# kowaalczyk/reformer-tts

Measured on AMD Instinct MI355X. Metric: mel-frames/sec training step, LJSpeech-shape batch, higher is better.
Workload: dtype bf16; 1 GPU; config/baseline.yml full Reformer-TTS training step (enc 3 / dec 3 layers, d=512, LSH 8 rounds, buckets 64/128), per-GPU batch 12, text 200->256, mel 1024x80; global_batch=12, parallelism=dp1, reversible_recompute=full

## Files before the change

### reformer-tts_amd/csrc/edges.hip

```cpp
#include "rtts_common.h"

#define ED_THREADS 256
#define ED_PBLOCKS 256

#define ed_drop rtts_drop_keep

struct EdHalo {
    int B, L, P, H;
};
__device__ __forceinline__ bool ed_valid(const EdHalo& g, long long m, int& b, int& t) {
    if (m < 0 || m >= (long long)g.B * g.P) return false;
    const int mi = (int)m;
    int q = (int)((float)mi * __builtin_amdgcn_rcpf((float)g.P));
    int r = mi - q * g.P;
    if (r < 0) { --q; r += g.P; }
    if (r >= g.P) { ++q; r -= g.P; }
    b = q;
    t = r - g.H;
    return (unsigned)t < (unsigned)g.L;
}
__device__ __forceinline__ void ed_row_col(unsigned e, int C, int cshift, unsigned& row, int& c) {
    if (cshift >= 0) {
        row = e >> cshift;
        c = (int)(e & (unsigned)(C - 1));
    } else {
        row = e / (unsigned)C;
        c = (int)(e - row * (unsigned)C);
    }
}
static inline int ed_cshift(int C) { return (C & (C - 1)) == 0 ? __builtin_ctz((unsigned)C) : -1; }
__device__ __forceinline__ float ed_tanh(float x) {
    const float t = __builtin_amdgcn_exp2f(x * 2.885390081777927f);
    return 1.f - 2.f * __builtin_amdgcn_rcpf(t + 1.f);
}
static inline EdHalo ed_halo(int B, int L, int halo) { return EdHalo{B, L, L + 2 * halo, halo}; }

template <bool SRC_F32>
__global__ __launch_bounds__(ED_THREADS) void to_halo_kernel(const void* __restrict__ src, int64_t ld_src, int64_t bs_src, int C_src, EdHalo g, int C,
                                                             int lead, long long rows, bf16_t* __restrict__ dst) {
    const int pieces = C / 8;
    const size_t total = (size_t)rows * pieces;
    for (size_t i = (size_t)blockIdx.x * blockDim.x + threadIdx.x; i < total; i += (size_t)gridDim.x * blockDim.x) {
        const int pc = (int)(i % pieces);
        const long long r = (long long)(i / pieces);
        int b, t;
        uint4 o = make_uint4(0, 0, 0, 0);
        if (pc * 8 < C_src && ed_valid(g, r - lead, b, t)) {
            const size_t soff = (size_t)b * bs_src + (size_t)t * ld_src;
            if (SRC_F32) {
                const float* p = reinterpret_cast<const float*>(src) + soff + pc * 8;
                const float4 v0 = *reinterpret_cast<const float4*>(p), v1 = *reinterpret_cast<const float4*>(p + 4);
                o.x = pack_bf16x2(v0.x, v0.y); o.y = pack_bf16x2(v0.z, v0.w);
                o.z = pack_bf16x2(v1.x, v1.y); o.w = pack_bf16x2(v1.z, v1.w);
            } else {
                o = *reinterpret_cast<const uint4*>(reinterpret_cast<const bf16_t*>(src) + soff + pc * 8);
            }
        }
        *reinterpret_cast<uint4*>(dst + (size_t)r * C + pc * 8) = o;
    }
}

__global__ __launch_bounds__(ED_THREADS) void conv_w_perm_kernel(const float* __restrict__ w, int Co, int Ci, int CP, bf16_t* __restrict__ wp) {
    const size_t total = (size_t)Co * 5 * CP;
    for (size_t i = (size_t)blockIdx.x * blockDim.x + threadIdx.x; i < total; i += (size_t)gridDim.x * blockDim.x) {
        const int ci = (int)(i % CP), k = (int)((i / CP) % 5), co = (int)(i / ((size_t)CP * 5));
        wp[i] = ci < Ci ? f32_to_bf16(w[((size_t)co * Ci + ci) * 5 + k]) : (bf16_t)0;
    }
}
struct CwGroup {
    rtts_conv_perm_job j[RTTS_CONV_PERM_MAX_GROUP];
    int blk_start[RTTS_CONV_PERM_MAX_GROUP + 1];
    int n;
};
__global__ __launch_bounds__(ED_THREADS) void conv_w_perm_grouped_kernel(const CwGroup g) {
    int ji = 0;
#pragma unroll
    for (int i = 1; i < RTTS_CONV_PERM_MAX_GROUP; ++i)
        if (i < g.n && (int)blockIdx.x >= g.blk_start[i]) ji = i;
    const rtts_conv_perm_job& J = g.j[ji];
    const int Co = J.Co, Ci = J.Ci, CP = J.CP;
    const float* __restrict__ w = J.w;
    bf16_t* __restrict__ wp = (bf16_t*)J.wp;
    const size_t total = (size_t)Co * CP;
    const size_t nthr = (size_t)(g.blk_start[ji + 1] - g.blk_start[ji]) * blockDim.x;
    for (size_t i = (size_t)((int)blockIdx.x - g.blk_start[ji]) * blockDim.x + threadIdx.x; i < total; i += nthr) {
        const int ci = (int)(i % CP), co = (int)(i / CP);
        float t[5] = {0.f, 0.f, 0.f, 0.f, 0.f};
        if (ci < Ci) {
            const float* src = w + ((size_t)co * Ci + ci) * 5;
#pragma unroll
            for (int k = 0; k < 5; ++k) t[k] = src[k];
        }
#pragma unroll
        for (int k = 0; k < 5; ++k) wp[((size_t)co * 5 + k) * CP + ci] = f32_to_bf16(t[k]);
    }
}
__global__ __launch_bounds__(ED_THREADS) void conv_dw_unperm_grouped_kernel(const CwGroup g) {
    int ji = 0;
#pragma unroll
    for (int i = 1; i < RTTS_CONV_PERM_MAX_GROUP; ++i)
        if (i < g.n && (int)blockIdx.x >= g.blk_start[i]) ji = i;
    const rtts_conv_perm_job& J = g.j[ji];
    const int Co = J.Co, Ci = J.Ci, CP = J.CP;
    const float* __restrict__ dwp = J.w;
    float* __restrict__ dw = (float*)J.wp;
    const size_t total = (size_t)Co * Ci;
    const size_t nthr = (size_t)(g.blk_start[ji + 1] - g.blk_start[ji]) * blockDim.x;
    for (size_t i = (size_t)((int)blockIdx.x - g.blk_start[ji]) * blockDim.x + threadIdx.x; i < total; i += nthr) {
        const int ci = (int)(i % Ci), co = (int)(i / Ci);
        float* dst = dw + i * 5;
#pragma unroll
        for (int k = 0; k < 5; ++k) dst[k] += dwp[((size_t)co * 5 + k) * CP + ci];
    }
}
__global__ __launch_bounds__(ED_THREADS) void conv_dw_unperm_kernel(const float* __restrict__ dwp, int Co, int Ci, int CP, float* __restrict__ dw) {
    const size_t total = (size_t)Co * Ci * 5;
    for (size_t i = (size_t)blockIdx.x * blockDim.x + threadIdx.x; i < total; i += (size_t)gridDim.x * blockDim.x) {
        const int k = (int)(i % 5), ci = (int)((i / 5) % Ci), co = (int)(i / ((size_t)Ci * 5));
        dw[i] += dwp[((size_t)co * 5 + k) * CP + ci];
    }
}

template <int MODE>
__global__ __launch_bounds__(ED_THREADS) void col_partial_kernel(const float* __restrict__ y, const bf16_t* __restrict__ dz,
                                                                 const float* __restrict__ mean, const float* __restrict__ rstd,
                                                                 const float* __restrict__ gamma, const float* __restrict__ beta, int act,
                                                                 uint32_t seed, const uint32_t* __restrict__ seed_dev, uint32_t thresh, float dscale, EdHalo g,
                                                                 int dz_halo, int C, float* __restrict__ partial) {
    if (seed_dev) seed += seed_dev[0];
    const int M = g.B * g.P;
    const int cq = threadIdx.x & 63, rl = threadIdx.x >> 6;
    const int c = blockIdx.y * 256 + cq * 4;
    __shared__ float red[2][4][256];
    float sa[4] = {0, 0, 0, 0}, sb[4] = {0, 0, 0, 0};
    if (c < C) {
        float mu[4] = {0, 0, 0, 0}, rs[4] = {1, 1, 1, 1}, ga[4] = {1, 1, 1, 1}, be[4] = {0, 0, 0, 0};
        if (MODE == 1) {
#pragma unroll
            for (int j = 0; j < 4; ++j) { mu[j] = mean[c + j]; rs[j] = rstd[c + j]; ga[j] = gamma[c + j]; be[j] = beta[c + j]; }
        }
        for (int row = blockIdx.x * 4 + rl; row < M; row += gridDim.x * 4) {
            int sb_, st_;
            if (!ed_valid(g, row, sb_, st_)) continue;
            const float4 yv = *reinterpret_cast<const float4*>(y + (size_t)row * C + c);
            const float yy[4] = {yv.x, yv.y, yv.z, yv.w};
            if (MODE == 0) {
#pragma unroll
                for (int j = 0; j < 4; ++j) { sa[j] += yy[j]; sb[j] = __builtin_fmaf(yy[j], yy[j], sb[j]); }
            } else {
                const size_t drow = dz_halo ? (size_t)row : (size_t)sb_ * g.L + st_;
                const uint2 dv = *reinterpret_cast<const uint2*>(dz + drow * C + c);
                const float dd[4] = {__uint_as_float(dv.x << 16), __uint_as_float(dv.x & 0xffff0000u), __uint_as_float(dv.y << 16),
                                     __uint_as_float(dv.y & 0xffff0000u)};
#pragma unroll
                for (int j = 0; j < 4; ++j) {
                    const float yh = (yy[j] - mu[j]) * rs[j];
                    const float pre = __builtin_fmaf(yh, ga[j], be[j]);
                    float da;
                    if (act == 1) da = pre > 0.f ? 1.f : 0.f;
                    else { const float th = ed_tanh(pre); da = 1.f - th * th; }
                    const float g = dd[j] * da * (thresh ? ed_drop(seed, (uint32_t)((size_t)row * C + c + j), thresh, dscale) : 1.f);
                    sa[j] += g;
                    sb[j] = __builtin_fmaf(g, yh, sb[j]);
                }
            }
        }
    }
#pragma unroll
    for (int j = 0; j < 4; ++j) { red[0][rl][cq * 4 + j] = sa[j]; red[1][rl][cq * 4 + j] = sb[j]; }
    __syncthreads();
    const int t = threadIdx.x;
    if (blockIdx.y * 256 + t < C) {
        float* prow = partial + (size_t)blockIdx.x * 2 * C;
        prow[blockIdx.y * 256 + t] = (red[0][0][t] + red[0][1][t]) + (red[0][2][t] + red[0][3][t]);
        prow[C + blockIdx.y * 256 + t] = (red[1][0][t] + red[1][1][t]) + (red[1][2][t] + red[1][3][t]);
    }
}

#define ED_FIN_WAVES 16
__device__ __forceinline__ void ed_reduce_partials(const float* __restrict__ partial, int nrows, int C, int c, float& s, float& q,
                                                   float (*red)[ED_FIN_WAVES][64]) {
    const int lane = threadIdx.x & 63, wave = threadIdx.x >> 6;
    float a = 0.f, b = 0.f;
    if (c < C) {
        float va[16], vb[16];
        for (int r0 = wave; r0 < nrows; r0 += ED_FIN_WAVES * 16) {
#pragma unroll
            for (int u = 0; u < 16; ++u) {
                const int r = r0 + u * ED_FIN_WAVES;
                va[u] = r < nrows ? partial[(size_t)r * 2 * C + c] : 0.f;
                vb[u] = r < nrows ? partial[(size_t)r * 2 * C + C + c] : 0.f;
            }
#pragma unroll
            for (int u = 0; u < 16; ++u) {
                a += va[u];
                b += vb[u];
            }
        }
    }
    red[0][wave][lane] = a;
    red[1][wave][lane] = b;
    __syncthreads();
    s = 0.f;
    q = 0.f;
#pragma unroll
    for (int w = 0; w < ED_FIN_WAVES; ++w) {
        s += red[0][w][lane];
        q += red[1][w][lane];
    }
}

__global__ __launch_bounds__(64 * ED_FIN_WAVES) void bn_finalize_stats_kernel(const float* __restrict__ partial, int nrows, int M, int C,
                                                                       float* __restrict__ mean, float* __restrict__ rstd,
                                                                       float* __restrict__ run_mean, float* __restrict__ run_var,
                                                                       const float* __restrict__ mean_shift, long long* __restrict__ num_batches) {
    __shared__ float red[2][ED_FIN_WAVES][64];
    const int c = blockIdx.x * 64 + (threadIdx.x & 63);
    float s, q;
    ed_reduce_partials(partial, nrows, C, c, s, q, red);
    if (num_batches && blockIdx.x == 0 && threadIdx.x == 0) num_batches[0] += 1;
    if (threadIdx.x >= 64 || c >= C) return;
    const float mu = s / M;
    const float var = fmaxf(q / M - mu * mu, 0.f);
    mean[c] = mu;
    rstd[c] = rsqrtf(var + 1e-5f);
    if (run_mean) {
        run_mean[c] = 0.9f * run_mean[c] + 0.1f * (mu + (mean_shift ? mean_shift[c] : 0.f));
        run_var[c] = 0.9f * run_var[c] + 0.1f * var * ((float)M / (float)(M > 1 ? M - 1 : 1));
    }
}

__global__ __launch_bounds__(64 * ED_FIN_WAVES) void bn_finalize_bwd_kernel(const float* __restrict__ partial, int nrows, int C,
                                                                     float* __restrict__ sums, float* __restrict__ dgamma,
                                                                     float* __restrict__ dbeta) {
    __shared__ float red[2][ED_FIN_WAVES][64];
    const int c = blockIdx.x * 64 + (threadIdx.x & 63);
    float s, q;
    ed_reduce_partials(partial, nrows, C, c, s, q, red);
    if (threadIdx.x >= 64 || c >= C) return;
    sums[c] = s;
    sums[C + c] = q;
    dbeta[c] += s;
    dgamma[c] += q;
}

__global__ __launch_bounds__(64 * ED_FIN_WAVES) void bn_moments_kernel(const float* __restrict__ partial, int nrows, int C, float* __restrict__ moments) {
    __shared__ float red[2][ED_FIN_WAVES][64];
    const int c = blockIdx.x * 64 + (threadIdx.x & 63);
    float s, q;
    ed_reduce_partials(partial, nrows, C, c, s, q, red);
    if (threadIdx.x >= 64 || c >= C) return;
    moments[c] = s;
    moments[C + c] = q;
}
__global__ void bn_from_moments_kernel(const float* __restrict__ moments, float count, int C, float* __restrict__ mean, float* __restrict__ rstd,
                                       float* __restrict__ run_mean, float* __restrict__ run_var, const float* __restrict__ mean_shift,
                                       long long* __restrict__ num_batches) {
    const int c = blockIdx.x * blockDim.x + threadIdx.x;
    if (num_batches && c == 0) num_batches[0] += 1;
    if (c >= C) return;
    if (count <= 0.f) count = moments[2 * C];
    const float mu = moments[c] / count;
    const float var = fmaxf(moments[C + c] / count - mu * mu, 0.f);
    mean[c] = mu;
    rstd[c] = rsqrtf(var + 1e-5f);
    if (run_mean) {
        run_mean[c] = 0.9f * run_mean[c] + 0.1f * (mu + (mean_shift ? mean_shift[c] : 0.f));
        run_var[c] = 0.9f * run_var[c] + 0.1f * var * (count / (count > 1.f ? count - 1.f : 1.f));
    }
}

__global__ __launch_bounds__(ED_THREADS) void bn_act_fwd_kernel(const float* __restrict__ y, const float* __restrict__ mean,
                                                                const float* __restrict__ rstd, const float* __restrict__ gamma,
                                                                const float* __restrict__ beta, int act, uint32_t seed, const uint32_t* __restrict__ seed_dev,
                                                                uint32_t thresh, float dscale, EdHalo g, int z_halo, int z_lead, size_t n4, int C,
                                                                int cshift, bf16_t* __restrict__ z) {
    if (seed_dev) seed += seed_dev[0];
    for (size_t i = (size_t)blockIdx.x * blockDim.x + threadIdx.x; i < n4; i += (size_t)gridDim.x * blockDim.x) {
        unsigned zrow;
        int c;
        ed_row_col((unsigned)i * 4u, C, cshift, zrow, c);
        const long long zr = (long long)zrow;
        long long ym;
        bool ok = true;
        if (z_halo) {
            int b, t;
            ym = zr - z_lead;
            ok = ed_valid(g, ym, b, t);
        } else {
            const long long b = zr / g.L;
            ym = b * g.P + g.H + (zr - b * g.L);
        }
        uint2 pk = make_uint2(0u, 0u);
        if (ok) {
            const size_t e = (size_t)ym * C + c;
            const float4 yv = *reinterpret_cast<const float4*>(y + e);
            const float yy[4] = {yv.x, yv.y, yv.z, yv.w};
            const float4 m4 = *reinterpret_cast<const float4*>(mean + c), r4 = *reinterpret_cast<const float4*>(rstd + c);
            const float4 g4 = *reinterpret_cast<const float4*>(gamma + c), b4 = *reinterpret_cast<const float4*>(beta + c);
            const float mu[4] = {m4.x, m4.y, m4.z, m4.w}, rs[4] = {r4.x, r4.y, r4.z, r4.w};
            const float ga[4] = {g4.x, g4.y, g4.z, g4.w}, be[4] = {b4.x, b4.y, b4.z, b4.w};
            float o[4];
#pragma unroll
            for (int j = 0; j < 4; ++j) {
                const float pre = __builtin_fmaf((yy[j] - mu[j]) * rs[j], ga[j], be[j]);
                float a = act == 1 ? fmaxf(pre, 0.f) : ed_tanh(pre);
                if (thresh) a *= ed_drop(seed, (uint32_t)(e + j), thresh, dscale);
                o[j] = a;
            }
            pk.x = pack_bf16x2(o[0], o[1]);
            pk.y = pack_bf16x2(o[2], o[3]);
        }
        reinterpret_cast<uint2*>(z)[i] = pk;
    }
}

__global__ __launch_bounds__(ED_THREADS) void bn_act_bwd_apply_kernel(const float* __restrict__ y, const bf16_t* __restrict__ dz,
                                                                      const float* __restrict__ mean, const float* __restrict__ rstd,
                                                                      const float* __restrict__ gamma, const float* __restrict__ beta, int act,
// ... 764 lines not shown
```

### reformer-tts_amd/csrc/fused_rows.hip

```cpp
#include "rtts_common.h"

#define FR_THREADS 256
#define FR_WAVES 4
#define FR_PARTIAL_BLOCKS 256

template <int VEC> struct VecF32;
template <> struct VecF32<2> { typedef float2 T; };
template <> struct VecF32<4> { typedef float4 T; };

template <int EPL, int VEC>
__device__ __forceinline__ void load_row_f32(const float* __restrict__ row, int lane, float* v) {
#pragma unroll
    for (int k = 0; k < EPL / VEC; ++k) {
        const typename VecF32<VEC>::T t = *reinterpret_cast<const typename VecF32<VEC>::T*>(row + (k * 64 + lane) * VEC);
        const float* f = reinterpret_cast<const float*>(&t);
#pragma unroll
        for (int j = 0; j < VEC; ++j) v[k * VEC + j] = f[j];
    }
}

template <int EPL, int VEC>
__device__ __forceinline__ void store_row_f32(float* __restrict__ row, int lane, const float* v) {
#pragma unroll
    for (int k = 0; k < EPL / VEC; ++k) {
        typename VecF32<VEC>::T t;
        float* f = reinterpret_cast<float*>(&t);
#pragma unroll
        for (int j = 0; j < VEC; ++j) f[j] = v[k * VEC + j];
        *reinterpret_cast<typename VecF32<VEC>::T*>(row + (k * 64 + lane) * VEC) = t;
    }
}

#ifndef RTTS_ROW_WT
#define RTTS_ROW_WT 0
#endif
template <int EPL, int VEC>
__device__ __forceinline__ void store_row_f32_out(float* __restrict__ row, int lane, const float* v) {
#if RTTS_ROW_WT >= 1
    if constexpr (VEC == 4) {
#pragma unroll
        for (int k = 0; k < EPL / VEC; ++k) {
            uint4 t;
            t.x = __float_as_uint(v[k * 4]); t.y = __float_as_uint(v[k * 4 + 1]); t.z = __float_as_uint(v[k * 4 + 2]); t.w = __float_as_uint(v[k * 4 + 3]);
            rtts_store16_out(row + (k * 64 + lane) * 4, t);
        }
        return;
    }
#endif
    store_row_f32<EPL, VEC>(row, lane, v);
}

template <int EPL, int VEC>
__device__ __forceinline__ void load_row_bf16(const bf16_t* __restrict__ row, int lane, float* v) {
#pragma unroll
    for (int k = 0; k < EPL / VEC; ++k) {
        const bf16_t* p = row + (k * 64 + lane) * VEC;
        if constexpr (VEC == 8) {
            const uint4 t = *reinterpret_cast<const uint4*>(p);
            const uint32_t u[4] = {t.x, t.y, t.z, t.w};
#pragma unroll
            for (int j = 0; j < 4; ++j) {
                v[k * 8 + 2 * j] = __uint_as_float(u[j] << 16);
                v[k * 8 + 2 * j + 1] = __uint_as_float(u[j] & 0xffff0000u);
            }
        } else if constexpr (VEC == 4) {
            const uint2 t = *reinterpret_cast<const uint2*>(p);
            v[k * 4] = __uint_as_float(t.x << 16);
            v[k * 4 + 1] = __uint_as_float(t.x & 0xffff0000u);
            v[k * 4 + 2] = __uint_as_float(t.y << 16);
            v[k * 4 + 3] = __uint_as_float(t.y & 0xffff0000u);
        } else {
            const uint32_t t = *reinterpret_cast<const uint32_t*>(p);
            v[k * 2] = __uint_as_float(t << 16);
            v[k * 2 + 1] = __uint_as_float(t & 0xffff0000u);
        }
    }
}

template <int EPL, int VEC, bool WT = true>
__device__ __forceinline__ void store_row_bf16(bf16_t* __restrict__ row, int lane, const float* v) {
#pragma unroll
    for (int k = 0; k < EPL / VEC; ++k) {
        bf16_t* p = row + (k * 64 + lane) * VEC;
        if constexpr (VEC == 8) {
            uint4 t;
            t.x = pack_bf16x2(v[k * 8], v[k * 8 + 1]);
            t.y = pack_bf16x2(v[k * 8 + 2], v[k * 8 + 3]);
            t.z = pack_bf16x2(v[k * 8 + 4], v[k * 8 + 5]);
            t.w = pack_bf16x2(v[k * 8 + 6], v[k * 8 + 7]);
            *reinterpret_cast<uint4*>(p) = t;
        } else if constexpr (VEC == 4) {
            uint2 t;
            t.x = pack_bf16x2(v[k * 4], v[k * 4 + 1]);
            t.y = pack_bf16x2(v[k * 4 + 2], v[k * 4 + 3]);
#if RTTS_ROW_WT >= 2
            if (WT) {
                typedef int rv2i __attribute__((ext_vector_type(2)));
                const rv2i w2 = {(int)t.x, (int)t.y};
                asm volatile("global_store_dwordx2 %0, %1, off sc1" ::"v"(p), "v"(w2) : "memory");
                continue;
            }
#endif
            *reinterpret_cast<uint2*>(p) = t;
        } else {
            *reinterpret_cast<uint32_t*>(p) = pack_bf16x2(v[k * 2], v[k * 2 + 1]);
        }
    }
}

template <int VEC>
__device__ __forceinline__ int row_col(int e, int lane) { return ((e / VEC) * 64 + lane) * VEC + (e % VEC); }

__device__ __forceinline__ float wave_sum(float s) {
#pragma unroll
    for (int o = 32; o > 0; o >>= 1) s += __shfl_xor(s, o);
    return s;
}

template <int EPL, int VEC>
__device__ __forceinline__ void block_partial(const float* acc, float* __restrict__ partial_row, float* lds) {
    const int lane = threadIdx.x & 63, wave = threadIdx.x >> 6;
    store_row_f32<EPL, VEC>(lds + wave * EPL * 64, lane, acc);
    __syncthreads();
    for (int c = threadIdx.x; c < EPL * 64; c += FR_THREADS)
        partial_row[c] = lds[c] + lds[EPL * 64 + c] + lds[2 * EPL * 64 + c] + lds[3 * EPL * 64 + c];
    __syncthreads();
}

template <int EPL, int VEC>
__global__ __launch_bounds__(FR_THREADS) void ln_fwd_kernel(const float* __restrict__ x, const float* __restrict__ gamma,
                                                            const float* __restrict__ beta, bf16_t* __restrict__ xn,
                                                            float* __restrict__ mean, float* __restrict__ rstd, int M) {
    constexpr int D = EPL * 64;
    const int lane = threadIdx.x & 63;
    const int row = blockIdx.x * FR_WAVES + (threadIdx.x >> 6);
    if (row >= M) return;
    float v[EPL], g[EPL], b[EPL];
    load_row_f32<EPL, VEC>(x + (size_t)row * D, lane, v);
    load_row_f32<EPL, VEC>(gamma, lane, g);
    load_row_f32<EPL, VEC>(beta, lane, b);
    float s = 0.f;
#pragma unroll
    for (int e = 0; e < EPL; ++e) s += v[e];
    const float mu = wave_sum(s) * (1.f / D);
    float q = 0.f;
#pragma unroll
    for (int e = 0; e < EPL; ++e) {
        v[e] -= mu;
        q = __builtin_fmaf(v[e], v[e], q);
    }
    const float rs = rsqrtf(wave_sum(q) * (1.f / D) + 1e-5f);
#pragma unroll
    for (int e = 0; e < EPL; ++e) v[e] = __builtin_fmaf(v[e] * rs, g[e], b[e]);
    store_row_bf16<EPL, VEC>(xn + (size_t)row * D, lane, v);
    if (lane == 0) {
        mean[row] = mu;
        rstd[row] = rs;
    }
}

template <int EPL, int VEC>
__global__ __launch_bounds__(FR_THREADS) void residual_ln_kernel(const float* x, float* y, const bf16_t* __restrict__ g,
                                                                 const float* __restrict__ bias, float sign,
                                                                 const float* __restrict__ gamma, const float* __restrict__ beta,
                                                                 bf16_t* __restrict__ xn, float* __restrict__ mean,
                                                                 float* __restrict__ rstd, int M, uint32_t seed,
                                                                 const uint32_t* __restrict__ seed_dev, uint32_t thresh, float dscale) {
    constexpr int D = EPL * 64;
    const int lane = threadIdx.x & 63;
    const int row = blockIdx.x * FR_WAVES + (threadIdx.x >> 6);
    if (row >= M) return;
    float v[EPL], gv[EPL], w[EPL];
    load_row_f32<EPL, VEC>(x + (size_t)row * D, lane, v);
    load_row_bf16<EPL, VEC>(g + (size_t)row * D, lane, gv);
    if (bias) {
        load_row_f32<EPL, VEC>(bias, lane, w);
#pragma unroll
        for (int e = 0; e < EPL; ++e) gv[e] += w[e];
    }
    if (thresh) {
        if (seed_dev) seed += seed_dev[0];
#pragma unroll
        for (int e = 0; e < EPL; ++e) gv[e] *= rtts_drop_keep(seed, (uint32_t)row * D + row_col<VEC>(e, lane), thresh, dscale);
    }
#pragma unroll
    for (int e = 0; e < EPL; ++e) v[e] += sign * gv[e];
    store_row_f32_out<EPL, VEC>(y + (size_t)row * D, lane, v);
    float s = 0.f;
#pragma unroll
    for (int e = 0; e < EPL; ++e) s += v[e];
    const float mu = wave_sum(s) * (1.f / D);
    float q = 0.f;
#pragma unroll
    for (int e = 0; e < EPL; ++e) {
        v[e] -= mu;
        q = __builtin_fmaf(v[e], v[e], q);
    }
    const float rs = rsqrtf(wave_sum(q) * (1.f / D) + 1e-5f);
    load_row_f32<EPL, VEC>(gamma, lane, gv);
    load_row_f32<EPL, VEC>(beta, lane, w);
#pragma unroll
    for (int e = 0; e < EPL; ++e) v[e] = __builtin_fmaf(v[e] * rs, gv[e], w[e]);
    store_row_bf16<EPL, VEC>(xn + (size_t)row * D, lane, v);
    if (lane == 0) {
        mean[row] = mu;
        rstd[row] = rs;
    }
}

template <int EPL, int VEC>
__global__ __launch_bounds__(FR_THREADS) void ln_bwd_kernel(const bf16_t* __restrict__ dxn, const float* __restrict__ x,
                                                            const float* __restrict__ mean, const float* __restrict__ rstd,
                                                            const float* __restrict__ gamma, const float* dx_in, const float* __restrict__ addend,
                                                            float* dx_io, float* __restrict__ partial_g, float* __restrict__ partial_b, int M,
                                                            bf16_t* __restrict__ dyb_next, float* __restrict__ partial_next,
                                                            uint32_t seed, const uint32_t* __restrict__ seed_dev, uint32_t thresh,
                                                            float dscale) {
    constexpr int D = EPL * 64;
    extern __shared__ __attribute__((aligned(16))) float lds_f[];
    const int lane = threadIdx.x & 63;
    float gam[EPL], ag[EPL], ab[EPL], an[EPL];
    load_row_f32<EPL, VEC>(gamma, lane, gam);
    if (thresh && seed_dev) seed += seed_dev[0];
#pragma unroll
    for (int e = 0; e < EPL; ++e) ag[e] = ab[e] = an[e] = 0.f;
    for (int row = blockIdx.x * FR_WAVES + (threadIdx.x >> 6); row < M; row += gridDim.x * FR_WAVES) {
        float dy[EPL], xv[EPL], dx[EPL];
        load_row_bf16<EPL, VEC>(dxn + (size_t)row * D, lane, dy);
        load_row_f32<EPL, VEC>(x + (size_t)row * D, lane, xv);
        load_row_f32<EPL, VEC>(dx_in + (size_t)row * D, lane, dx);
        if (addend) {
            float ad[EPL];
            load_row_f32<EPL, VEC>(addend + (size_t)row * D, lane, ad);
#pragma unroll
            for (int e = 0; e < EPL; ++e) dx[e] += ad[e];
        }
        const float mu = mean[row], rs = rstd[row];
        float s1 = 0.f, s2 = 0.f;
#pragma unroll
        for (int e = 0; e < EPL; ++e) {
            xv[e] = (xv[e] - mu) * rs;
            ag[e] = __builtin_fmaf(dy[e], xv[e], ag[e]);
            ab[e] += dy[e];
            dy[e] *= gam[e];
            s1 += dy[e];
            s2 = __builtin_fmaf(dy[e], xv[e], s2);
        }
        s1 = wave_sum(s1) * (1.f / D);
        s2 = wave_sum(s2) * (1.f / D);
#pragma unroll
        for (int e = 0; e < EPL; ++e) dx[e] += rs * (dy[e] - s1 - xv[e] * s2);
        store_row_f32_out<EPL, VEC>(dx_io + (size_t)row * D, lane, dx);
        if (dyb_next) {
            if (thresh) {
#pragma unroll
                for (int e = 0; e < EPL; ++e) dx[e] *= rtts_drop_keep(seed, (uint32_t)row * D + row_col<VEC>(e, lane), thresh, dscale);
            }
#pragma unroll
            for (int e = 0; e < EPL; ++e) an[e] += dx[e];
            store_row_bf16<EPL, VEC>(dyb_next + (size_t)row * D, lane, dx);
        }
    }
    block_partial<EPL, VEC>(ag, partial_g + (size_t)blockIdx.x * D, lds_f);
    block_partial<EPL, VEC>(ab, partial_b + (size_t)blockIdx.x * D, lds_f);
    if (dyb_next) block_partial<EPL, VEC>(an, partial_next + (size_t)blockIdx.x * D, lds_f);
}

template <int EPL, int VEC>
__global__ __launch_bounds__(FR_THREADS) void cast_colsum_kernel(const float* __restrict__ dy, bf16_t* __restrict__ dyb,
                                                                 float* __restrict__ partial, int M, uint32_t seed,
                                                                 const uint32_t* __restrict__ seed_dev, uint32_t thresh, float dscale,
                                                                 const float* __restrict__ scale_dev) {
    constexpr int D = EPL * 64;
    extern __shared__ __attribute__((aligned(16))) float lds_f[];
    const int lane = threadIdx.x & 63;
    float acc[EPL];
#pragma unroll
    for (int e = 0; e < EPL; ++e) acc[e] = 0.f;
    if (thresh && seed_dev) seed += seed_dev[0];
    const float up = scale_dev ? scale_dev[0] : 1.f;
    for (int row = blockIdx.x * FR_WAVES + (threadIdx.x >> 6); row < M; row += gridDim.x * FR_WAVES) {
        float v[EPL];
        load_row_f32<EPL, VEC>(dy + (size_t)row * D, lane, v);
        if (scale_dev) {
#pragma unroll
            for (int e = 0; e < EPL; ++e) v[e] *= up;
        }
        if (thresh) {
#pragma unroll
            for (int e = 0; e < EPL; ++e) v[e] *= rtts_drop_keep(seed, (uint32_t)row * D + row_col<VEC>(e, lane), thresh, dscale);
        }
#pragma unroll
        for (int e = 0; e < EPL; ++e) acc[e] += v[e];
        store_row_bf16<EPL, VEC>(dyb + (size_t)row * D, lane, v);
    }
    block_partial<EPL, VEC>(acc, partial + (size_t)blockIdx.x * D, lds_f);
}

template <int EPL, int VEC, bool RELU>
__global__ __launch_bounds__(FR_THREADS) void colsum_bf16_kernel(const bf16_t* dh, const bf16_t* __restrict__ h, bf16_t* dst,
                                                                 int64_t ld, float* __restrict__ partial, int M, float gate_scale) {
    constexpr int D = EPL * 64;
    constexpr int AV = (EPL % 4 == 0) ? 4 : 2;
    extern __shared__ __attribute__((aligned(16))) float lds_f[];
    const int lane = threadIdx.x & 63;
    float acc[EPL];
#pragma unroll
    for (int e = 0; e < EPL; ++e) acc[e] = 0.f;
    for (int row = blockIdx.x * FR_WAVES + (threadIdx.x >> 6); row < M; row += gridDim.x * FR_WAVES) {
        float v[EPL];
        load_row_bf16<EPL, VEC>(dh + (size_t)row * ld, lane, v);
        if (RELU) {
            float hv[EPL];
            load_row_bf16<EPL, VEC>(h + (size_t)row * ld, lane, hv);
#pragma unroll
            for (int e = 0; e < EPL; ++e) v[e] = hv[e] > 0.f ? v[e] * gate_scale : 0.f;
            store_row_bf16<EPL, VEC>(dst + (size_t)row * ld, lane, v);
        }
#pragma unroll
        for (int e = 0; e < EPL; ++e) acc[e] += v[e];
    }
    const int wave = threadIdx.x >> 6;
#pragma unroll
    for (int k = 0; k < EPL / VEC; ++k)
#pragma unroll
        for (int j = 0; j < VEC; ++j) lds_f[wave * D + (k * 64 + lane) * VEC + j] = acc[k * VEC + j];
    __syncthreads();
    float* prow = partial + (size_t)blockIdx.x * D;
    for (int c = threadIdx.x; c < D; c += FR_THREADS) prow[c] = lds_f[c] + lds_f[D + c] + lds_f[2 * D + c] + lds_f[3 * D + c];
    (void)AV;
}

__global__ __launch_bounds__(FR_THREADS) void colsum_final_kernel(const float* __restrict__ partial, int nrows, int n,
                                                                  float* __restrict__ out, const float* __restrict__ partial2,
                                                                  float* __restrict__ out2) {
    __shared__ float red[FR_WAVES][64];
    if (blockIdx.y) {
        partial = partial2;
        out = out2;
    }
    const int lane = threadIdx.x & 63, wave = threadIdx.x >> 6;
    const int c = blockIdx.x * 64 + lane;
    float s = 0.f;
    if (c < n) {
#pragma unroll 8
        for (int r = wave; r < nrows; r += FR_WAVES) s += partial[(size_t)r * n + c];
    }
    red[wave][lane] = s;
    __syncthreads();
    if (wave == 0 && c < n) out[c] += (red[0][lane] + red[1][lane]) + (red[2][lane] + red[3][lane]);
}

struct CsJob {
    const float* partial;
    float* out;
    int nrows, n, ld, blk_start;
};
struct CsGroup {
    CsJob j[RTTS_COLSUM_MAX_GROUP];
    int n;
};
#define CS_WAVES 16
__global__ __launch_bounds__(64 * CS_WAVES) void colsum_final_grouped_kernel(const CsGroup grp) {
    __shared__ float red[CS_WAVES][64];
    int ji = 0;
#pragma unroll 1
    for (int i = 1; i < grp.n; ++i)
        if ((int)blockIdx.x >= grp.j[i].blk_start) ji = i;
    const CsJob& J = grp.j[ji];
    const int lane = threadIdx.x & 63, wave = threadIdx.x >> 6;
    const int c = ((int)blockIdx.x - J.blk_start) * 64 + lane;
    float s = 0.f;
    if (c < J.n) {
        float v[16];
#pragma unroll
        for (int k = 0; k < 16; ++k) {
            const int r = wave + k * CS_WAVES;
            v[k] = r < J.nrows ? J.partial[(size_t)r * J.ld + c] : 0.f;
        }
#pragma unroll
        for (int k = 0; k < 16; k += 4) s += (v[k] + v[k + 1]) + (v[k + 2] + v[k + 3]);
        for (int r = wave + 16 * CS_WAVES; r < J.nrows; r += CS_WAVES) s += J.partial[(size_t)r * J.ld + c];
    }
    red[wave][lane] = s;
    __syncthreads();
    if (wave == 0 && c < J.n) {
        float t = 0.f;
#pragma unroll
        for (int w = 0; w < CS_WAVES; w += 4) t += (red[w][lane] + red[w + 1][lane]) + (red[w + 2][lane] + red[w + 3][lane]);
        J.out[c] += t;
    }
}

__global__ __launch_bounds__(FR_THREADS) void residual_epilogue_kernel(const float* __restrict__ x, const bf16_t* __restrict__ g,
                                                                       const float* __restrict__ bias, float sign,
                                                                       float* __restrict__ y, size_t n4, int d, uint32_t seed,
                                                                       const uint32_t* __restrict__ seed_dev, uint32_t thresh,
                                                                       float dscale) {
    if (thresh && seed_dev) seed += seed_dev[0];
    for (size_t i = (size_t)blockIdx.x * blockDim.x + threadIdx.x; i < n4; i += (size_t)gridDim.x * blockDim.x) {
        const float4 xv = reinterpret_cast<const float4*>(x)[i];
        const uint2 gv = reinterpret_cast<const uint2*>(g)[i];
        float4 bv = make_float4(0.f, 0.f, 0.f, 0.f);
        if (bias) bv = *reinterpret_cast<const float4*>(bias + (i * 4) % d);
        float f[4] = {__uint_as_float(gv.x << 16) + bv.x, __uint_as_float(gv.x & 0xffff0000u) + bv.y,
                      __uint_as_float(gv.y << 16) + bv.z, __uint_as_float(gv.y & 0xffff0000u) + bv.w};
        if (thresh) {
#pragma unroll
            for (int j = 0; j < 4; ++j) f[j] *= rtts_drop_keep(seed, (uint32_t)(i * 4 + j), thresh, dscale);
        }
        float4 o;
        o.x = xv.x + sign * f[0];
        o.y = xv.y + sign * f[1];
        o.z = xv.z + sign * f[2];
        o.w = xv.w + sign * f[3];
        reinterpret_cast<float4*>(y)[i] = o;
    }
}

__global__ __launch_bounds__(FR_THREADS) void bias_act_kernel(bf16_t* __restrict__ h, const float* __restrict__ bias, size_t n8, int d,
                                                              int relu) {
    for (size_t i = (size_t)blockIdx.x * blockDim.x + threadIdx.x; i < n8; i += (size_t)gridDim.x * blockDim.x) {
        uint4 t = reinterpret_cast<uint4*>(h)[i];
        const float* b = bias + (i * 8) % d;
        const float4 b0 = *reinterpret_cast<const float4*>(b), b1 = *reinterpret_cast<const float4*>(b + 4);
        uint32_t u[4] = {t.x, t.y, t.z, t.w};
        const float bb[8] = {b0.x, b0.y, b0.z, b0.w, b1.x, b1.y, b1.z, b1.w};
#pragma unroll
        for (int j = 0; j < 4; ++j) {
            float lo = __uint_as_float(u[j] << 16) + bb[2 * j], hi = __uint_as_float(u[j] & 0xffff0000u) + bb[2 * j + 1];
            if (relu) {
                lo = fmaxf(lo, 0.f);
                hi = fmaxf(hi, 0.f);
            }
            u[j] = pack_bf16x2(lo, hi);
        }
        t.x = u[0]; t.y = u[1]; t.z = u[2]; t.w = u[3];
        reinterpret_cast<uint4*>(h)[i] = t;
    }
}

__global__ __launch_bounds__(FR_THREADS) void cast_f32_bf16_kernel(const float* __restrict__ src, bf16_t* __restrict__ dst, size_t n4) {
    for (size_t i = (size_t)blockIdx.x * blockDim.x + threadIdx.x; i < n4; i += (size_t)gridDim.x * blockDim.x) {
        const float4 v = reinterpret_cast<const float4*>(src)[i];
        uint2 o;
        o.x = pack_bf16x2(v.x, v.y);
        o.y = pack_bf16x2(v.z, v.w);
        reinterpret_cast<uint2*>(dst)[i] = o;
    }
}

static inline unsigned stream_grid(size_t work_items) {
    size_t b = (work_items + FR_THREADS - 1) / FR_THREADS;
    if (b > 4096) b = 4096;
    if (b < 1) b = 1;
    return (unsigned)b;
}

#define FR_DISPATCH_D(d, CALL)                                    \
    switch (d) {                                                  \
        case 128: { CALL(2, 2); break; }                          \
        case 256: { CALL(4, 4); break; }                          \
        case 384: { CALL(6, 2); break; }                          \
        case 512: { CALL(8, 4); break; }                          \
        case 768: { CALL(12, 4); break; }                         \
        case 1024: { CALL(16, 4); break; }                        \
        case 2048: { CALL(32, 4); break; }                        \
        default:                                                  \
            rtts_set_error("row kernels: width %d unsupported (128, 256, 384, 512, 768, 1024, 2048)", d); \
            return -1;                                            \
    }

extern "C" int rtts_ln_fwd(const float* x, const float* gamma, const float* beta, void* xn, float* mean, float* rstd, int M, int d,
                           void* stream) {
    RTTS_ENTER(stream);
// ... 187 lines not shown
```

### reformer-tts_amd/csrc/rtts_common.h

```cpp
#pragma once
#include <hip/hip_runtime.h>
#include <stdint.h>
#include <stdio.h>
#include <stdarg.h>
#include <atomic>

#include "../../include/rtts.h"

typedef uint16_t bf16_t;
typedef __attribute__((ext_vector_type(8))) __bf16 bf16x8;
typedef __attribute__((ext_vector_type(4))) __bf16 bf16x4;
typedef __attribute__((ext_vector_type(4))) short short4v;
typedef __attribute__((ext_vector_type(16))) float f32x16;
typedef __attribute__((ext_vector_type(4))) float f32x4;

#define RTTS_LDS __attribute__((address_space(3)))

extern "C" void rtts_set_error(const char* fmt, ...);
int rtts_walk_override(int backward);

#define RTTS_REQUIRE(cond, ...)            \
    do {                                   \
        if (!(cond)) {                     \
            rtts_set_error(__VA_ARGS__);   \
            return -1;                     \
        }                                  \
    } while (0)

#define RTTS_LAUNCH_CHECK(name)                                              \
    do {                                                                     \
        hipError_t e_ = hipGetLastError();                                   \
        if (e_ != hipSuccess) {                                              \
            int dev_ = -1;                                                   \
            (void)hipGetDevice(&dev_);                                       \
            rtts_set_error("%s: launch failed: %s (current device %d; the entry points launch on the caller's current device: " \
                           "the stream and every pointer must belong to it)", name, hipGetErrorString(e_), dev_); \
            return -2;                                                       \
        }                                                                    \
    } while (0)

static inline int rtts_bind_device(void* stream) {
    if (!stream) return 0;
    hipDevice_t dev = -1;
    if (hipStreamGetDevice((hipStream_t)stream, &dev) != hipSuccess) {
        (void)hipGetLastError();
        rtts_set_error("the stream handle %p does not belong to any device of this process", stream);
        return -3;
    }
    int cur = -1;
    if (hipGetDevice(&cur) == hipSuccess && cur == (int)dev) return 0;
    if (hipSetDevice((int)dev) != hipSuccess) {
        (void)hipGetLastError();
        rtts_set_error("cannot bind the calling thread to device %d (the device of the stream)", (int)dev);
        return -3;
    }
    return 0;
}
#define RTTS_ENTER(stream)                              \
    do {                                                \
        const int rc_enter_ = rtts_bind_device(stream); \
        if (rc_enter_) return rc_enter_;                \
    } while (0)

struct RttsLdsState { std::atomic<size_t> set[64]; };
static inline hipError_t rtts_ensure_lds(const void* func, size_t lds, RttsLdsState& st) {
    if (lds <= 64 * 1024) return hipSuccess;
    int dev = 0;
    if (hipGetDevice(&dev) != hipSuccess || dev < 0 || dev >= 64) dev = 0;
    if (st.set[dev].load(std::memory_order_acquire) >= lds) return hipSuccess;
    const hipError_t e = hipFuncSetAttribute(func, hipFuncAttributeMaxDynamicSharedMemorySize, (int)lds);
    if (e == hipSuccess) {
        size_t cur = st.set[dev].load(std::memory_order_relaxed);
        while (cur < lds && !st.set[dev].compare_exchange_weak(cur, lds, std::memory_order_release, std::memory_order_relaxed)) {}
    }
    return e;
}
#define RTTS_ENSURE_LDS(name, func, lds, state)                                                                   \
    do {                                                                                                          \
        const hipError_t e_lds_ = rtts_ensure_lds(reinterpret_cast<const void*>(func), (lds), (state));           \
        RTTS_REQUIRE(e_lds_ == hipSuccess, "%s: cannot raise the dynamic LDS limit to %zu bytes: %s", name, (size_t)(lds), \
                     hipGetErrorString(e_lds_));                                                                  \
    } while (0)

#ifndef RTTS_WT_STORES
#define RTTS_WT_STORES 1
#endif
typedef int rtts_v4i __attribute__((ext_vector_type(4)));
__device__ __forceinline__ void rtts_store16_out(void* p, const uint4 v) {
#if RTTS_WT_STORES
    const rtts_v4i w = {(int)v.x, (int)v.y, (int)v.z, (int)v.w};
    asm volatile("global_store_dwordx4 %0, %1, off sc1\n\ts_nop 1" ::"v"(p), "v"(w) : "memory");
#else
    *reinterpret_cast<uint4*>(p) = v;
#endif
}

__device__ __forceinline__ float bf16_to_f32(bf16_t x) { return __uint_as_float(((uint32_t)x) << 16); }

__device__ __forceinline__ bf16_t f32_to_bf16(float x) {
    __bf16 b = (__bf16)x;
    return __builtin_bit_cast(bf16_t, b);
}

typedef __attribute__((ext_vector_type(2))) float f32x2;
typedef __attribute__((ext_vector_type(8))) float f32x8;
typedef __attribute__((ext_vector_type(2))) __bf16 bf16x2;

__device__ __forceinline__ uint32_t pack_bf16x2(float lo, float hi) {
    const f32x2 v = {lo, hi};
    return __builtin_bit_cast(uint32_t, __builtin_convertvector(v, bf16x2));
}

__device__ __forceinline__ bf16x8 cvt_bf16x8(float a0, float a1, float a2, float a3, float a4, float a5, float a6, float a7) {
    const f32x8 v = {a0, a1, a2, a3, a4, a5, a6, a7};
    return __builtin_convertvector(v, bf16x8);
}

__device__ __forceinline__ float rtts_sum8(float x) {
    x += __int_as_float(__builtin_amdgcn_update_dpp(0, __float_as_int(x), 0xB1, 0xF, 0xF, true));
    x += __int_as_float(__builtin_amdgcn_update_dpp(0, __float_as_int(x), 0x4E, 0xF, 0xF, true));
    x += __int_as_float(__builtin_amdgcn_update_dpp(0, __float_as_int(x), 0x141, 0xF, 0xF, true));
    return x;
}
__device__ __forceinline__ float rtts_xhalf_sum(float x) {
    const auto r = __builtin_amdgcn_permlane32_swap(__float_as_uint(x), __float_as_uint(x), false, false);
    return __uint_as_float(r[0]) + __uint_as_float(r[1]);
}
__device__ __forceinline__ float rtts_xhalf_max(float x) {
    const auto r = __builtin_amdgcn_permlane32_swap(__float_as_uint(x), __float_as_uint(x), false, false);
    return fmaxf(__uint_as_float(r[0]), __uint_as_float(r[1]));
}

#define RTTS_LSH_BWD_QK_SLOTS 2

__device__ __forceinline__ uint32_t xcd_remap(uint32_t id, uint32_t n) {
    const uint32_t q = n >> 3, r = n & 7u, x = id & 7u, i = id >> 3;
    return (x < r ? x * (q + 1) : r * (q + 1) + (x - r) * q) + i;
}

__device__ __forceinline__ uint32_t rtts_drop_hash(uint32_t seed, uint32_t idx) {
    uint32_t s = seed;
    s ^= s >> 16; s *= 0x85ebca6bu; s ^= s >> 13; s *= 0xc2b2ae35u; s ^= s >> 16;
    uint32_t x = idx * 0x9E3779B1u + s;
    x ^= x >> 16; x *= 0x7feb352du; x ^= (s << 13) | (s >> 19); x ^= x >> 15; x *= 0x846ca68bu; x ^= x >> 16;
    return x;
}
__device__ __forceinline__ float rtts_drop_keep(uint32_t seed, uint32_t idx, uint32_t thresh, float scale) {
    return rtts_drop_hash(seed, idx) >= thresh ? scale : 0.f;
}
static inline uint32_t rtts_drop_thresh(float p) { return p <= 0.f ? 0u : (uint32_t)((double)p * 4294967296.0); }
```

Baseline: 1.949 million mel-frames/s.

## Software-pipeline row loads in reduction and layernorm-backward kernels

```diff
diff --git a/reformer-tts_amd/csrc/edges.hip b/reformer-tts_amd/csrc/edges.hip
--- a/reformer-tts_amd/csrc/edges.hip
+++ b/reformer-tts_amd/csrc/edges.hip
@@ -139,17 +139,29 @@
 #pragma unroll
             for (int j = 0; j < 4; ++j) { mu[j] = mean[c + j]; rs[j] = rstd[c + j]; ga[j] = gamma[c + j]; be[j] = beta[c + j]; }
         }
-        for (int row = blockIdx.x * 4 + rl; row < M; row += gridDim.x * 4) {
+        constexpr int P = MODE == 0 ? 6 : 4;
+        float4 yr[P];
+        uint2 dzr[P];
+        bool ok[P];
+        auto issue = [&](int s, int r, bool live) __attribute__((always_inline)) {
             int sb_, st_;
-            if (!ed_valid(g, row, sb_, st_)) continue;
-            const float4 yv = *reinterpret_cast<const float4*>(y + (size_t)row * C + c);
+            ok[s] = live && ed_valid(g, r, sb_, st_);
+            if (!ok[s]) { r = g.H; sb_ = 0; st_ = 0; }
+            yr[s] = *reinterpret_cast<const float4*>(y + (size_t)r * C + c);
+            if (MODE == 1) {
+                const size_t drow = dz_halo ? (size_t)r : (size_t)sb_ * g.L + st_;
+                dzr[s] = *reinterpret_cast<const uint2*>(dz + drow * C + c);
+            }
+        };
+        auto process = [&](int s, int row) __attribute__((always_inline)) {
+            if (!ok[s]) return;
+            const float4 yv = yr[s];
             const float yy[4] = {yv.x, yv.y, yv.z, yv.w};
             if (MODE == 0) {
 #pragma unroll
                 for (int j = 0; j < 4; ++j) { sa[j] += yy[j]; sb[j] = __builtin_fmaf(yy[j], yy[j], sb[j]); }
             } else {
-                const size_t drow = dz_halo ? (size_t)row : (size_t)sb_ * g.L + st_;
-                const uint2 dv = *reinterpret_cast<const uint2*>(dz + drow * C + c);
+                const uint2 dv = dzr[s];
                 const float dd[4] = {__uint_as_float(dv.x << 16), __uint_as_float(dv.x & 0xffff0000u), __uint_as_float(dv.y << 16),
                                      __uint_as_float(dv.y & 0xffff0000u)};
 #pragma unroll
@@ -164,7 +176,8 @@
                     sb[j] = __builtin_fmaf(g, yh, sb[j]);
                 }
             }
-        }
+        };
+        rtts_row_pipeline<P>(blockIdx.x * 4 + __builtin_amdgcn_readfirstlane(rl), gridDim.x * 4, M, issue, process);
     }
 #pragma unroll
     for (int j = 0; j < 4; ++j) { red[0][rl][cq * 4 + j] = sa[j]; red[1][rl][cq * 4 + j] = sb[j]; }
diff --git a/reformer-tts_amd/csrc/fused_rows.hip b/reformer-tts_amd/csrc/fused_rows.hip
--- a/reformer-tts_amd/csrc/fused_rows.hip
+++ b/reformer-tts_amd/csrc/fused_rows.hip
@@ -75,6 +75,36 @@
             v[k * 2 + 1] = __uint_as_float(t & 0xffff0000u);
         }
     }
+}
+
+template <int EPL, int VEC>
+__device__ __forceinline__ void load_row_bf16_raw(const bf16_t* row, int lane, uint32_t* raw) {
+#pragma unroll
+    for (int k = 0; k < EPL / VEC; ++k) {
+        const bf16_t* p = row + (k * 64 + lane) * VEC;
+        if constexpr (VEC == 8) {
+            const uint4 t = *reinterpret_cast<const uint4*>(p);
+            raw[k * 4] = t.x; raw[k * 4 + 1] = t.y; raw[k * 4 + 2] = t.z; raw[k * 4 + 3] = t.w;
+        } else if constexpr (VEC == 4) {
+            const uint2 t = *reinterpret_cast<const uint2*>(p);
+            raw[k * 2] = t.x; raw[k * 2 + 1] = t.y;
+        } else {
+            raw[k] = *reinterpret_cast<const uint32_t*>(p);
+        }
+    }
+}
+template <int EPL>
+__device__ __forceinline__ void unpack_row_bf16(const uint32_t* raw, float* v) {
+#pragma unroll
+    for (int w = 0; w < EPL / 2; ++w) {
+        v[2 * w] = __uint_as_float(raw[w] << 16);
+        v[2 * w + 1] = __uint_as_float(raw[w] & 0xffff0000u);
+    }
+}
+
+__host__ __device__ constexpr int fr_depth(int row_bytes) {
+    const int p = (12288 + row_bytes - 1) / row_bytes;
+    return p < 2 ? 2 : (p > 6 ? 6 : p);
 }
 
 template <int EPL, int VEC, bool WT = true>
@@ -217,6 +247,7 @@
                                                             uint32_t seed, const uint32_t* __restrict__ seed_dev, uint32_t thresh,
                                                             float dscale) {
     constexpr int D = EPL * 64;
+    constexpr int P = EPL >= 32 ? 1 : fr_depth(EPL * 64 * 10);
     extern __shared__ __attribute__((aligned(16))) float lds_f[];
     const int lane = threadIdx.x & 63;
     float gam[EPL], ag[EPL], ab[EPL], an[EPL];
@@ -224,18 +255,32 @@
     if (thresh && seed_dev) seed += seed_dev[0];
 #pragma unroll
     for (int e = 0; e < EPL; ++e) ag[e] = ab[e] = an[e] = 0.f;
-    for (int row = blockIdx.x * FR_WAVES + (threadIdx.x >> 6); row < M; row += gridDim.x * FR_WAVES) {
+    const int wave = __builtin_amdgcn_readfirstlane(threadIdx.x >> 6);
+    const int vzero = (int)(threadIdx.x >> 6) - wave;
+    uint32_t dyr[P][EPL / 2];
+    float xr[P][EPL], dr[P][EPL], ar[P][EPL], mur[P], rsr[P];
+    auto issue = [&](int s, int r, bool live) __attribute__((always_inline)) {
+        const int ln = live ? lane : 0;
+        load_row_bf16_raw<EPL, VEC>(dxn + (size_t)r * D, ln, dyr[s]);
+        load_row_f32<EPL, VEC>(x + (size_t)r * D, ln, xr[s]);
+        load_row_f32<EPL, VEC>(dx_in + (size_t)r * D, ln, dr[s]);
+        if (addend) load_row_f32<EPL, VEC>(addend + (size_t)r * D, ln, ar[s]);
+        mur[s] = mean[r + vzero];
+        rsr[s] = rstd[r + vzero];
+    };
+    auto process = [&](int s, int row) __attribute__((always_inline)) {
         float dy[EPL], xv[EPL], dx[EPL];
-        load_row_bf16<EPL, VEC>(dxn + (size_t)row * D, lane, dy);
-        load_row_f32<EPL, VEC>(x + (size_t)row * D, lane, xv);
-        load_row_f32<EPL, VEC>(dx_in + (size_t)row * D, lane, dx);
+        unpack_row_bf16<EPL>(dyr[s], dy);
+#pragma unroll
+        for (int e = 0; e < EPL; ++e) {
+            xv[e] = xr[s][e];
+            dx[e] = dr[s][e];
+        }
         if (addend) {
-            float ad[EPL];
-            load_row_f32<EPL, VEC>(addend + (size_t)row * D, lane, ad);
-#pragma unroll
-            for (int e = 0; e < EPL; ++e) dx[e] += ad[e];
-        }
-        const float mu = mean[row], rs = rstd[row];
+#pragma unroll
+            for (int e = 0; e < EPL; ++e) dx[e] += ar[s][e];
+        }
+        const float mu = mur[s], rs = rsr[s];
         float s1 = 0.f, s2 = 0.f;
 #pragma unroll
         for (int e = 0; e < EPL; ++e) {
@@ -260,7 +305,8 @@
             for (int e = 0; e < EPL; ++e) an[e] += dx[e];
             store_row_bf16<EPL, VEC>(dyb_next + (size_t)row * D, lane, dx);
         }
-    }
+    };
+    rtts_row_pipeline<P>(blockIdx.x * FR_WAVES + wave, gridDim.x * FR_WAVES, M, issue, process);
     block_partial<EPL, VEC>(ag, partial_g + (size_t)blockIdx.x * D, lds_f);
     block_partial<EPL, VEC>(ab, partial_b + (size_t)blockIdx.x * D, lds_f);
     if (dyb_next) block_partial<EPL, VEC>(an, partial_next + (size_t)blockIdx.x * D, lds_f);
@@ -279,9 +325,16 @@
     for (int e = 0; e < EPL; ++e) acc[e] = 0.f;
     if (thresh && seed_dev) seed += seed_dev[0];
     const float up = scale_dev ? scale_dev[0] : 1.f;
-    for (int row = blockIdx.x * FR_WAVES + (threadIdx.x >> 6); row < M; row += gridDim.x * FR_WAVES) {
+    constexpr int P = fr_depth(EPL * 64 * 4);
+    const int wave = __builtin_amdgcn_readfirstlane(threadIdx.x >> 6);
+    float vr[P][EPL];
+    auto issue = [&](int s, int r, bool live) __attribute__((always_inline)) {
+        load_row_f32<EPL, VEC>(dy + (size_t)r * D, live ? lane : 0, vr[s]);
+    };
+    auto process = [&](int s, int row) __attribute__((always_inline)) {
         float v[EPL];
-        load_row_f32<EPL, VEC>(dy + (size_t)row * D, lane, v);
+#pragma unroll
+        for (int e = 0; e < EPL; ++e) v[e] = vr[s][e];
         if (scale_dev) {
 #pragma unroll
             for (int e = 0; e < EPL; ++e) v[e] *= up;
@@ -293,7 +346,8 @@
 #pragma unroll
         for (int e = 0; e < EPL; ++e) acc[e] += v[e];
         store_row_bf16<EPL, VEC>(dyb + (size_t)row * D, lane, v);
-    }
+    };
+    rtts_row_pipeline<P>(blockIdx.x * FR_WAVES + wave, gridDim.x * FR_WAVES, M, issue, process);
     block_partial<EPL, VEC>(acc, partial + (size_t)blockIdx.x * D, lds_f);
 }
 
@@ -307,20 +361,28 @@
     float acc[EPL];
 #pragma unroll
     for (int e = 0; e < EPL; ++e) acc[e] = 0.f;
-    for (int row = blockIdx.x * FR_WAVES + (threadIdx.x >> 6); row < M; row += gridDim.x * FR_WAVES) {
+    constexpr int P = fr_depth(EPL * 64 * (RELU ? 4 : 2));
+    uint32_t dr[P][EPL / 2], hr[P][EPL / 2];
+    auto issue = [&](int s, int r, bool live) __attribute__((always_inline)) {
+        const int ln = live ? lane : 0;
+        load_row_bf16_raw<EPL, VEC>(dh + (size_t)r * ld, ln, dr[s]);
+        if (RELU) load_row_bf16_raw<EPL, VEC>(h + (size_t)r * ld, ln, hr[s]);
+    };
+    auto process = [&](int s, int row) __attribute__((always_inline)) {
         float v[EPL];
-        load_row_bf16<EPL, VEC>(dh + (size_t)row * ld, lane, v);
+        unpack_row_bf16<EPL>(dr[s], v);
         if (RELU) {
             float hv[EPL];
-            load_row_bf16<EPL, VEC>(h + (size_t)row * ld, lane, hv);
+            unpack_row_bf16<EPL>(hr[s], hv);
 #pragma unroll
             for (int e = 0; e < EPL; ++e) v[e] = hv[e] > 0.f ? v[e] * gate_scale : 0.f;
             store_row_bf16<EPL, VEC>(dst + (size_t)row * ld, lane, v);
         }
 #pragma unroll
         for (int e = 0; e < EPL; ++e) acc[e] += v[e];
-    }
-    const int wave = threadIdx.x >> 6;
+    };
+    const int wave = __builtin_amdgcn_readfirstlane(threadIdx.x >> 6);
+    rtts_row_pipeline<P>(blockIdx.x * FR_WAVES + wave, gridDim.x * FR_WAVES, M, issue, process);
 #pragma unroll
     for (int k = 0; k < EPL / VEC; ++k)
 #pragma unroll
diff --git a/reformer-tts_amd/csrc/rtts_common.h b/reformer-tts_amd/csrc/rtts_common.h
--- a/reformer-tts_amd/csrc/rtts_common.h
+++ b/reformer-tts_amd/csrc/rtts_common.h
@@ -149,3 +149,27 @@
     return rtts_drop_hash(seed, idx) >= thresh ? scale : 0.f;
 }
 static inline uint32_t rtts_drop_thresh(float p) { return p <= 0.f ? 0u : (uint32_t)((double)p * 4294967296.0); }
+
+template <int P, class Issue, class Process>
+__device__ __forceinline__ void rtts_row_pipeline(int row0, int stride, int M, Issue issue, Process process) {
+    if (row0 >= M) return;
+#pragma unroll
+    for (int s = 0; s < P - 1; ++s) {
+        const int r = row0 + s * stride;
+        issue(s, r < M ? r : row0, r < M);
+    }
+    int base = row0;
+    for (; base + (P - 1) * stride < M; base += P * stride) {
+#pragma unroll
+        for (int s = 0; s < P; ++s) {
+            const int row = base + s * stride, rn = row + (P - 1) * stride;
+            issue((s + P - 1) % P, rn < M ? rn : row0, rn < M);
+            process(s, row);
+        }
+    }
+#pragma unroll
+    for (int s = 0; s < P - 1; ++s) {
+        if (base + s * stride >= M) return;
+        process(s, base + s * stride);
+    }
+}
```

Measured after the change: 1.962 million mel-frames/s (median of 6 runs). About the same (+0.6%).
